# apapiu/transformer_latent_diffusion

Measured on AMD Instinct MI355X. Metric: images/sec (256px, 35-step CFG sampling), denoiser only, higher is better.
Workload: dtype bf16; 1 GPU; C1: 100M-param denoiser (d=768, L=12), 32x32x4 latents, 35 steps + CFG 6, DPM-Solver++(2M), 64 images/GPU (model batch 128); images_per_gpu=64, global_batch=64, n_iter=35, parallelism=single GPU

## Files before the change

### transformer_latent_diffusion_amd/csrc/tld_common.h

```cpp
#pragma once
#include <hip/hip_runtime.h>
#include <atomic>
#include <mutex>
#include <stdint.h>
#include "tld_gemm_plan.h"

namespace tld {

typedef __attribute__((ext_vector_type(8))) __bf16 bf16x8;
typedef __attribute__((ext_vector_type(4))) __bf16 bf16x4;
typedef __attribute__((ext_vector_type(2))) __bf16 bf16x2;
typedef __attribute__((ext_vector_type(16))) float f32x16;
typedef __attribute__((ext_vector_type(4))) float f32x4;
typedef __attribute__((ext_vector_type(4))) unsigned u32x4;
typedef __attribute__((ext_vector_type(8))) int i32x8;
typedef __attribute__((ext_vector_type(2))) float f32x2;

constexpr int kWave = 64;
constexpr int kHeadDim = 64;
constexpr float kLnEps = 1e-5f;

template <int CTRL>
__device__ __forceinline__ float dpp_add(float v) {
    const int s = __builtin_amdgcn_update_dpp(0, __float_as_int(v), CTRL, 0xf, 0xf, true);
// ... 222 lines not shown
    }
    return c;
}

enum : int {
    EP_EMBED_PLAIN = 0, EP_EMBED_MFMA = 1 , EP_LN_Q4 = 5 , EP_LN_GENERIC = 9, EP_LN_MX8 = 10,
    EP_QKV_ATTN = 11, EP_QKV_LN = 12, EP_QKV_PLAIN = 13,
    EP_ATT_256 = 14, EP_ATT_CHUNKED = 15, EP_ATT_64 = 17 , EP_ATT_MASKED = 19,
    EP_CROSS_MFMA = 20 , EP_CROSS_GPW1 = 24, EP_CROSS_GPWN = 25, EP_CROSS_VALU = 26, EP_CROSS_FANOUT = 27,
    EP_UP_FUSED16 = 28, EP_UP_FUSED32_SEAM = 29, EP_UP_FUSED16_SMALL = 30, EP_UP_PLAIN = 31, EP_DW_WHOLE = 32, EP_DW_TILED = 33, EP_DW_STREAM = 34,
    EP_DOWN_STATS = 35, EP_DOWN_NOSTATS = 36, EP_DOWN_MAIN = 37, EP_DOWN_SMALL64 = 38, EP_DOWN_SMALL128 = 39,
    EP_SPLITK4 = 40, EP_SPLITK8 = 41, EP_SPLITK_SMALL = 42, EP_SPLITK_FINISH12 = 43, EP_SPLITK_FINISH6 = 44,
    EP_TAIL_MFMA = 45 , EP_TAIL_PLAIN = 49, EP_UPDATE = 50, EP_UPDATE_FROM = 51, EP_UPDATE_FROM_MASK = 52, EP_START_MIX = 53,
    EP_QUANT_MX8 = 54, EP_CROSS_F8 = 55, EP_DW_TILED_F8 = 56, EP_DW_STREAM_F8 = 57,
    EP_UPDATE_REQ = 58, EP_UPDATE_REQ_MASK = 59, EP_START_MIX_REQ = 60,
    EP_COUNT = 61
};
extern thread_local uint64_t* g_path_sink;
inline void note_path(int bit) { if (g_path_sink) *g_path_sink |= 1ull << bit; }

int launch_gemm(const GemmParams& p, int epilogue, hipStream_t s);
void launch_updw_pp(const GemmParams& p, const GemmPlan& plan, hipStream_t s);
void launch_splitk_pp(const GemmParams& p, const GemmPlan& plan, hipStream_t s);
void launch_down_pp(const GemmParams& p, const GemmPlan& plan, hipStream_t s);
void launch_dwconv_seam(const uint32_t* seam, const uint32_t* dw_wpk, const float* dw_b_half, bf16* out, int ldo, int batch, int channels, hipStream_t s);
void launch_gemm_tn(const GemmParams& p, hipStream_t s);

void set_last_error(const char* msg);

void launch_quant_mx8(const bf16* in, uint8_t* out, uint8_t* scale, int M, int K, hipStream_t s);
// ... 50 lines not shown
    float* sa_out;
    int batch, ntok, d, heads;
};
void launch_cross_row(const CrossRowParams& p, hipStream_t s);
bool cross_row_supports_ln3_stats(int d);
bool splitk_resid_supported(int d);
void launch_splitk_resid(const float* parts, int nsplit, size_t slice_stride, const float* bias, resid_t* x, float2* stats_out, int M, int d, hipStream_t s);

struct TailParams {
    const resid_t* tok;
    const float* w;
    const bf16* w_hl;
    const float* b;
    float* out;
    int batch, C, S, p, grid, pd, d, ntok;
};
void launch_tail(const TailParams& p, hipStream_t s);

struct SamplerStepRow {
    float g, a, b, c, c1, c2;
    float s_next;
    int final_step;
};
struct SamplerStepParams {
    const float* x0_2b;
    float* x_t;
    float* x0_prev;
    float* out_latent;
    float* trace_x0; float* trace_xt;
    const float* noise;
    const float* z0;
    const float* mask;
// ... 25 lines not shown
```

### transformer_latent_diffusion_amd/csrc/tld_engine.hip

```cpp
#include "../../include/tld_hip.h"
#include "tld_common.h"
#include "tld_host.h"
#include "tld_refresh.h"

#include <cmath>
#include <cstdarg>
#include <cstdio>
#include <cstring>
#include <cstdlib>
#include <map>
#include <string>
#include <unordered_map>
#include <vector>

using namespace tld;

namespace {
thread_local char g_err[512] = "";
}
namespace tld {
void set_last_error(const char* msg) { snprintf(g_err, sizeof(g_err), "%s", msg); }
thread_local uint64_t* g_path_sink = nullptr;
}
namespace {
// ... 8 lines not shown
    tld_config cfg{};
    int d = 0, L = 0, H = 0, ntok = 0, grid = 0, pd = 0, hid = 0, img = 0, ne = 0, text = 0;
    bool finalized = false;
    bool fuse_dwconv = true;
    bool fp8 = false;
    bool fp8_fused = true;
    uint8_t *a8 = nullptr, *as8 = nullptr;
    std::map<std::string, HostTensor> host;

    float *angular = nullptr, *ff1_w = nullptr, *ff1_b = nullptr, *ff3_w = nullptr, *ff3_b = nullptr;
    float *label_w = nullptr, *label_b = nullptr, *norm_w = nullptr, *norm_b = nullptr;
    float *conv_w = nullptr, *conv_b = nullptr, *pln1_w = nullptr, *pln1_b = nullptr, *plin_wt = nullptr,
          *plin_b = nullptr, *pln2_w = nullptr, *pln2_b = nullptr, *pos = nullptr, *out_w = nullptr,
          *out_b = nullptr;
    bf16* out_w_hl = nullptr;
    bf16* plin_w_hl = nullptr;
    std::vector<Layer> layers;
    const float **tab_kv_w = nullptr, **tab_q_w = nullptr, **tab_n2_w = nullptr, **tab_n2_b = nullptr;
    RefreshPlan refresh;
    int64_t nparam = 0;

    resid_t* x = nullptr;
    resid_t* x_half = nullptr;
    bool share_l0 = true;
    bool guidance_skip = true;
    int64_t rows_cond = 0, rows_uncond = 0;
    bool fold_ln1 = true;
    bool low_latency = false;
    float* splitk = nullptr;
    int ll_split = 0;
// ... 119 lines not shown

#define SNAP(...) do { if (e->dbg_keep) { if (int _r = e->stages.copy(__VA_ARGS__)) return _r; } } while (0)
inline std::string blk_name(int l, const char* n) { return "blk" + std::to_string(l) + "." + n; }

inline bool eng_fused_qa(const tld_engine* e) { return e->fuse_qkv_attn && e->fold_ln1 && !e->fp8; }
inline bool eng_fuse_dw(const tld_engine* e) { return e->fuse_dwconv && (e->grid == 16 || (e->grid == 32 && e->seam)) && e->hid % 256 == 0; }

int reserve_snapshots(tld_engine* e) {
    const size_t B = (size_t)e->cfg.max_batch, M = B * e->ntok, d = e->d, hid = e->hid;
#define RES(name, bytes) do { if (int _r = e->stages.reserve(name, bytes)) return _r; } while (0)
    const size_t rs = sizeof(resid_t);
    RES("tokens0", M * d * rs); RES("out", B * e->img * 4);
    for (const char* n : {"step.x_t", "step.x0_prev", "step.x0", "step.x_next"}) RES(n, B * e->img * 4);
    RES("step.out", B * e->img * 4);
    for (int l = 0; l < e->L; ++l) {
        for (const char* n : {"x_in", "ca", "mlp"}) RES(blk_name(l, n), M * d * rs);
        RES(blk_name(l, "att"), M * d * 2); RES(blk_name(l, "sa"), M * d * 4);
        if (e->fold_ln1) RES(blk_name(l, "ln1"), M * kLnSlots * 8); else RES(blk_name(l, "xn1"), M * d * 2);
        if (!eng_fused_qa(e)) { RES(blk_name(l, "qk"), M * 2 * d * 2); RES(blk_name(l, "vt"), M * d * 2); }
        if (e->fold_ln3) RES(blk_name(l, "stats"), M * 8); else RES(blk_name(l, "xn3"), M * d * 2);
        if (!eng_fuse_dw(e)) RES(blk_name(l, "hid_pre"), M * hid * 2);
        if (e->fp8) {
            RES(blk_name(l, "a8_qkv.q"), M * d); RES(blk_name(l, "a8_qkv.s"), M * d / 32);
            RES(blk_name(l, "a8_up.q"), M * d); RES(blk_name(l, "a8_up.s"), M * d / 32);
            RES(blk_name(l, "a8_down.q"), M * hid); RES(blk_name(l, "a8_down.s"), M * hid / 32);
        }
        RES(blk_name(l, "hid"), M * hid * 2);
        if (e->splitk) RES(blk_name(l, "splitk"), (size_t)e->ll_split * M * d * 4);
    }
#undef RES
    for (int l = 0; l < e->L; ++l) {
// ... 196 lines not shown
                if (fold3) {
                    g.A = e->x; g.W = Ly.up_wf; g.bias = Ly.up_b1; g.ln_c1 = Ly.up_c1; g.row_stats = e->row_stats;
                }
#endif
                GEMM_TRY(blk_name(l, "up-projection"), launch_gemm(g, EPI_BIAS_BF16, s));
            }
            SNAP(blk_name(l, "hid_pre"), e->hid1, ST_BF16, s, M, e->hid);
            {
                ProfScope ps(e, KC_DWCONV, s);
                const bool dw8 = fuse8 && e->grid > 16;
                launch_dwconv_gelu(e->hid1, e->hid2, Ly.dw_w9c, Ly.dw_b, Ly.dw_w9c_half, Ly.dw_b_half, batch, e->grid, e->hid, s,
                                   dw8 ? e->a8 : nullptr, dw8 ? e->as8 : nullptr);
            }
        }
        if (!(fuse8 && e->grid > 16)) SNAP(blk_name(l, "hid"), e->hid2, ST_BF16, s, M, e->hid);
        if (e->low_latency && !e->fp8) {
            ProfScope ps(e, KC_GEMM_DOWN, s);
            GemmParams g{};
            g.A = e->hid2; g.lda = e->hid; g.W = Ly.down_w; g.ldw = e->hid; g.M = M; g.N = d; g.K = e->hid / e->ll_split; g.ksplit = e->ll_split;
            g.c_f32 = e->splitk; g.ldc = d;
            GEMM_TRY(blk_name(l, "split-K down projection"), launch_gemm(g, EPI_F32, s));
            SNAP(blk_name(l, "splitk"), e->splitk, ST_F32, s, e->ll_split, M, d);
            launch_splitk_resid(e->splitk, e->ll_split, (size_t)M * d, Ly.down_b, e->x, (fold1 && l + 1 < e->L) ? e->ln_stats : nullptr, M, d, s);
        } else
        {
            ProfScope ps(e, KC_GEMM_DOWN, s);
            GemmParams g{};
            g.A = e->hid2; g.lda = e->hid; g.W = Ly.down_w; g.ldw = e->hid; g.M = M; g.N = d; g.K = e->hid;
            g.bias = Ly.down_b; g.resid = e->x; g.ldr = d;
            g.stats_out = (fold1 && l + 1 < e->L) ? e->ln_stats : nullptr;
            if (e->fp8) {
                if (!(fuse8 && e->grid > 16)) launch_quant_mx8(e->hid2, e->a8, e->as8, M, e->hid, s);
                SNAP(blk_name(l, "a8_down.q"), e->a8, ST_U8, s, M, e->hid); SNAP(blk_name(l, "a8_down.s"), e->as8, ST_MX8S, s, M, e->hid / 32);
                g.f8 = 1; g.A = reinterpret_cast<const bf16*>(e->a8); g.W = reinterpret_cast<const bf16*>(Ly.down_w8);
                g.a_scale = e->as8; g.w_scale = Ly.down_s8;
            }
            GEMM_TRY(blk_name(l, "down projection"), launch_gemm(g, EPI_BIAS_RESID, s));
        }
        SNAP(blk_name(l, "mlp"), e->x, rdt, s, M, d);
    }
    {
        ProfScope ps(e, KC_TAIL, s);
        TailParams tp{};
        tp.tok = e->x; tp.w = e->out_w; tp.w_hl = e->out_w_hl; tp.b = e->out_b; tp.out = out; tp.batch = batch;
        tp.C = e->cfg.n_channels; tp.S = e->cfg.image_size; tp.p = e->cfg.patch_size; tp.grid = e->grid;
        tp.pd = e->pd; tp.d = d; tp.ntok = e->ntok;
        launch_tail(tp, s);
    }
    SNAP("out", out, ST_F32, s, batch, e->img);
    HIP_TRY(hipGetLastError());
    return TLD_OK;
}

struct SamplePlan {
    int B, n_max, stride;
    const tld_sample_request* requests;
    const float* coeffs;
    const float* guidance;
    int Tn; const float* sig; const int* noise_idx;
    const float *noise, *init_latent, *mask, *labels, *neg_labels;
    float sharp, bright;
// ... 194 lines not shown
    if (strncmp(prop.gcnArchName, "gfx950", 6) != 0)
        return fail(TLD_ERR_INVALID, "device %d is %s; this engine is built for gfx950 only", c->device_id, prop.gcnArchName);
    tld_engine* e = new tld_engine();
    e->cfg = *c;
    e->d = c->embed_dim; e->L = c->n_layers; e->H = c->embed_dim / 64; e->grid = grid; e->ntok = ntok;
    e->pd = pd; e->hid = c->mlp_multiplier * c->embed_dim; e->img = c->n_channels * c->image_size * c->image_size;
    e->ne = c->noise_embed_dims; e->text = c->text_emb_size;
    e->layers.resize(e->L);
    e->nparam = make_param_layout(e->d, e->L, e->ne, e->pd, e->hid, e->ntok, e->text).count;
    if (const char* fd = getenv("TLD_FUSE_DWCONV")) e->fuse_dwconv = atoi(fd) != 0;
    if (const char* sl = getenv("TLD_SHARE_L0")) e->share_l0 = atoi(sl) != 0;
    if (const char* gs = getenv("TLD_GUIDANCE_SKIP")) e->guidance_skip = atoi(gs) != 0;
    if (const char* f8 = getenv("TLD_FP8_FUSED")) e->fp8_fused = atoi(f8) != 0;
    if (const char* fl = getenv("TLD_FOLD_LN3")) e->fold_ln3 = atoi(fl) != 0;
    if (const char* fl = getenv("TLD_FOLD_LN1")) e->fold_ln1 = atoi(fl) != 0;
#ifndef TLD_RESID_BF16
    e->fold_ln3 = false;
    e->fold_ln1 = false;
#endif
    e->fold_ln1 = e->fold_ln1 && gemm_resid_stat_slots(e->d) > 0 && (3 * e->d) % 256 == 0;
    e->fold_ln3 = e->fold_ln3 && e->hid % 256 == 0 && cross_row_supports_ln3_stats(e->d);
    if (const char* fq = getenv("TLD_FUSE_QKV_ATTN")) e->fuse_qkv_attn = atoi(fq) != 0;
    e->fuse_qkv_attn = e->fuse_qkv_attn && e->fold_ln1 && ntok == 256 && e->d % 128 == 0;
    *out = e;
    return TLD_OK;
}

int tld_engine_load_tensor(tld_engine* e, const char* key, const void* host_ptr, const int64_t* shape,
                           int32_t ndim, int32_t dtype) {
    if (!e || !key || (!host_ptr && ndim > 0)) return fail(TLD_ERR_INVALID, "null argument");
    if (e->finalized) return fail(TLD_ERR_STATE, "weights already finalized");
// ... 209 lines not shown
                for (int64_t c = 0; c < hid; ++c) {
                    const uint32_t w0 = f32_to_bf16_rne(tr[(size_t)((du * 3 + 0) * hid + c)]);
                    const uint32_t w1 = f32_to_bf16_rne(tr[(size_t)((du * 3 + 1) * hid + c)]);
                    const uint32_t w2 = f32_to_bf16_rne(tr[(size_t)((du * 3 + 2) * hid + c)]);
                    pk[(size_t)((du * 4 + 0) * hid + c)] = w0 << 16;
                    pk[(size_t)((du * 4 + 1) * hid + c)] = w1 | (w2 << 16);
                    pk[(size_t)((du * 4 + 2) * hid + c)] = w0 | (w1 << 16);
                    pk[(size_t)((du * 4 + 3) * hid + c)] = w2;
                }
            if (int rc = dev_alloc(e, &Ly.dw_wpk, pk.size())) return rc;
            HIP_TRY(hipMemcpy(Ly.dw_wpk, pk.data(), pk.size() * sizeof(uint32_t), hipMemcpyHostToDevice));
            e->weight_bytes += (int64_t)pk.size() * 4;
        }
#undef LK
    }
    e->host.clear();
    {
        const size_t L = (size_t)e->L;
        std::vector<const float*> hk(L), hq(L), hg(L), hb(L);
        for (size_t l = 0; l < L; ++l) { hk[l] = e->layers[l].kv_w; hq[l] = e->layers[l].q_w; hg[l] = e->layers[l].n2_w; hb[l] = e->layers[l].n2_b; }
        const float** tabs = nullptr;
        if (int rc = dev_alloc(e, &tabs, 4 * L)) return rc;
        e->tab_kv_w = tabs; e->tab_q_w = tabs + L; e->tab_n2_w = tabs + 2 * L; e->tab_n2_b = tabs + 3 * L;
        HIP_TRY(hipMemcpy(e->tab_kv_w, hk.data(), L * sizeof(float*), hipMemcpyHostToDevice));
        HIP_TRY(hipMemcpy(e->tab_q_w, hq.data(), L * sizeof(float*), hipMemcpyHostToDevice));
        HIP_TRY(hipMemcpy(e->tab_n2_w, hg.data(), L * sizeof(float*), hipMemcpyHostToDevice));
        HIP_TRY(hipMemcpy(e->tab_n2_b, hb.data(), L * sizeof(float*), hipMemcpyHostToDevice));
    }
    {
        const ParamLayout pl = make_param_layout(e->d, e->L, e->ne, e->pd, e->hid, e->ntok, e->text);
// ... 2 lines not shown
        R.d = e->d; R.hid = e->hid; R.L = e->L; R.l0 = pl.layers[0]; R.layer_stride = pl.layer_stride();
        R.fold = e->fold_ln1 || e->fold_ln3; R.fp8 = e->fp8;
        Layer* ld = nullptr;
        if (int rc = dev_alloc(e, &ld, (size_t)e->L)) return rc;
        HIP_TRY(hipMemcpy(ld, e->layers.data(), (size_t)e->L * sizeof(Layer), hipMemcpyHostToDevice));
        R.layers_dev = ld;
        auto job = [&R](void* dst, int64_t src, int64_t n, int kind = RJ_COPY, int cols = 0) { if (dst) R.jobs[R.njobs++] = RefreshJob{dst, src, n, kind, cols}; };
        job(e->ff1_w, pl.ff1w, d * ne); job(e->ff1_b, pl.ff1b, d); job(e->ff3_w, pl.ff3w, d * d); job(e->ff3_b, pl.ff3b, d);
        job(e->label_w, pl.lbw, d * text); job(e->label_b, pl.lbb, d); job(e->norm_w, pl.nw, d); job(e->norm_b, pl.nb, d);
        job(e->conv_w, pl.cvw, pd * cpp); job(e->conv_b, pl.cvb, pd); job(e->pln1_w, pl.l1w, pd); job(e->pln1_b, pl.l1b, pd);
        job(e->plin_b, pl.lib, d); job(e->pln2_w, pl.l2w, d); job(e->pln2_b, pl.l2b, d); job(e->pos, pl.pos, N * d);
        job(e->out_w, pl.outw, pd * d); job(e->out_b, pl.outb, pd);
        job(e->out_w_hl, pl.outw, pd * d, RJ_SPLIT_HL); job(e->plin_w_hl, pl.liw, d * pd, RJ_SPLIT_HL);
        job(e->plin_wt, pl.liw, d * pd, RJ_TRANSPOSE, (int)pd);
        static_assert(kRefreshMaxJobs >= 21, "the images outside the blocks");
    }

    const size_t B2 = (size_t)e->cfg.max_batch, M = B2 * e->ntok;
    if (int rc = dev_alloc(e, &e->x, M * d)) return rc;
    if (int rc = dev_alloc(e, &e->x_half, M * d)) return rc;
    if (int rc = dev_alloc(e, &e->xn, M * d)) return rc;
    if (int rc = dev_alloc(e, &e->row_stats, M + 256)) return rc;
    if (int rc = dev_alloc(e, &e->ln_stats, (M + 256) * kLnSlots)) return rc;
    if (int rc = dev_alloc(e, &e->qk, M * 2 * d)) return rc;
    if (int rc = dev_alloc(e, &e->vt, M * d)) return rc;
    if (int rc = dev_alloc(e, &e->att, M * d)) return rc;
    if (int rc = dev_alloc(e, &e->hid1, M * hid)) return rc;
    if (e->grid == 32 && e->fuse_dwconv && hid % 256 == 0) { if (int rc = dev_alloc(e, &e->seam, M * hid / 4)) return rc; }
    if (int rc = dev_alloc(e, &e->hid2, M * hid)) return rc;
    if (e->fp8) {
// ... 552 lines not shown
```

### transformer_latent_diffusion_amd/csrc/tld_refresh.h

```cpp
#pragma once

#include "tld_param_layout.h"

namespace tld {

struct Layer {
    bf16 *qkv_w = nullptr, *up_w = nullptr, *down_w = nullptr;
    bf16 *qkv_wf = nullptr;
    float *qkv_c1 = nullptr, *qkv_b1 = nullptr;
    bf16 *qkv_wp = nullptr;
    float *qkv_c1p = nullptr, *qkv_b1p = nullptr;
    float *up_b = nullptr, *dw_w9c = nullptr, *dw_b = nullptr, *down_b = nullptr;
    float *dw_w9c_half = nullptr, *dw_b_half = nullptr;
    uint32_t* dw_wpk = nullptr;
    uint8_t *qkv_w8 = nullptr, *qkv_s8 = nullptr, *up_w8 = nullptr, *up_s8 = nullptr, *down_w8 = nullptr, *down_s8 = nullptr;
    bf16 *up_wf = nullptr;
    float *up_c1 = nullptr, *up_b1 = nullptr;
    float *n1_w = nullptr, *n1_b = nullptr, *n2_w = nullptr, *n2_b = nullptr, *n3_w = nullptr, *n3_b = nullptr;
    float *kv_w = nullptr, *q_w = nullptr;
};

enum { RJ_COPY = 0,
       RJ_SPLIT_HL = 1,
       RJ_TRANSPOSE = 2 };
struct RefreshJob { void* dst; int64_t src, n; int32_t kind, cols; };
constexpr int kRefreshMaxJobs = 24;

struct RefreshPlan {
    int d = 0, hid = 0, L = 0;
    const Layer* layers_dev = nullptr;
    LayerOffsets l0{};
    int64_t layer_stride = 0;
    bool fold = false, fp8 = false;
    RefreshJob jobs[kRefreshMaxJobs];
    int njobs = 0;
};

int launch_refresh_weights(const RefreshPlan& p, const float* flat, hipStream_t s);
void launch_quant_mx8_f32(const float* in, uint8_t* out, uint8_t* scale, int rows, int K, hipStream_t s);

}
```

### transformer_latent_diffusion_amd/csrc/tld_refresh.hip

```cpp
#include "tld_common.h"
#include "tld_stages.h"
#include "tld_refresh.h"
#include "tld_refresh_math.h"

namespace tld {

namespace {

struct RefreshJobs { RefreshJob job[kRefreshMaxJobs]; };

__device__ __forceinline__ uint16_t bf16_bits(float f) { return bf16_rne_bits(__float_as_uint(f)); }
__device__ __forceinline__ float bf16_value(uint16_t h) { return __uint_as_float((uint32_t)h << 16); }

__device__ __forceinline__ void copy_f32(float* __restrict__ dst, const float* __restrict__ src, int64_t n, int64_t tid, int64_t nth) {
    if (((reinterpret_cast<uintptr_t>(src) | reinterpret_cast<uintptr_t>(dst)) & 15) == 0 && (n & 3) == 0) {
        const float4* s4 = reinterpret_cast<const float4*>(src);
        float4* d4 = reinterpret_cast<float4*>(dst);
        for (int64_t i = tid; i < (n >> 2); i += nth) d4[i] = s4[i];
    } else {
        for (int64_t i = tid; i < n; i += nth) dst[i] = src[i];
    }
}

__device__ __forceinline__ void cast_bf16(uint16_t* __restrict__ dst, const float* __restrict__ src, int64_t n, int64_t tid, int64_t nth) {
// ... 123 lines not shown
            const float w = tile[lane][k];
            const float qf = bf16_value(bf16_bits(gs[k] * w));
            sc += (double)qf;
            sb += (double)bs[k] * (double)w;
        }
        __syncthreads();
    }
    const int n = row0 + lane;
    const float c1 = (float)sc;
    const float b1 = ln3 ? (float)(sb + (double)base[o.up_b + n]) : (float)sb;
    (ln3 ? Ly.up_c1 : Ly.qkv_c1)[n] = c1;
    (ln3 ? Ly.up_b1 : Ly.qkv_b1)[n] = b1;
    if (wp) { Ly.qkv_c1p[packed_row(lane)] = c1; Ly.qkv_b1p[packed_row(lane)] = b1; }
}

__device__ __forceinline__ void quant_mx8_f32_rows(const float* __restrict__ in, uint8_t* __restrict__ out, uint8_t* __restrict__ scale, int rows, int K,
                                                   int64_t tid, int64_t nth) {
    const int gpr = K >> 3;
    const int64_t groups = (int64_t)rows * gpr;
    const bool vec = (reinterpret_cast<uintptr_t>(in) & 15) == 0;
    for (int64_t g = tid; g < groups; g += nth) {
        const int row = (int)(g / gpr), k0 = (int)(g - (int64_t)row * gpr) * 8;
        const float* p = in + (int64_t)row * K + k0;
        float f[8];
        if (vec) {
            const float4 a = *reinterpret_cast<const float4*>(p), b = *reinterpret_cast<const float4*>(p + 4);
            f[0] = a.x; f[1] = a.y; f[2] = a.z; f[3] = a.w; f[4] = b.x; f[5] = b.y; f[6] = b.z; f[7] = b.w;
        } else {
#pragma unroll
            for (int e = 0; e < 8; ++e) f[e] = p[e];
// ... 33 lines not shown
    else if (blockIdx.y == 1) { if (Ly.up_w8) quant_mx8_f32_rows(base + o.up_w, Ly.up_w8, Ly.up_s8, hid, d, tid, nth); }
    else if (Ly.down_w8) quant_mx8_f32_rows(base + o.down_w, Ly.down_w8, Ly.down_s8, d, hid, tid, nth);
}

}

int launch_refresh_weights(const RefreshPlan& p, const float* flat, hipStream_t s) {
    RefreshJobs J{};
    for (int i = 0; i < p.njobs; ++i) J.job[i] = p.jobs[i];
    hipLaunchKernelGGL(refresh_globals_kernel, dim3(64, (unsigned)p.njobs), dim3(256), 0, s, J, flat);
    hipLaunchKernelGGL(refresh_layer_kernel, dim3(32, LJ_COUNT, (unsigned)p.L), dim3(256), 0, s, p.layers_dev, flat, p.l0, p.layer_stride, p.d, p.hid);
    if (p.fold) {
        const int rows = p.hid > 3 * p.d ? p.hid : 3 * p.d;
        hipLaunchKernelGGL(refresh_fold_kernel, dim3((unsigned)(rows / 64), 2, (unsigned)p.L), dim3(64), 0, s, p.layers_dev, flat, p.l0, p.layer_stride, p.d, p.hid);
    }
    if (p.fp8) hipLaunchKernelGGL(refresh_fp8_kernel, dim3(64, 3, (unsigned)p.L), dim3(256), 0, s, p.layers_dev, flat, p.l0, p.layer_stride, p.d, p.hid);
    const hipError_t e = hipGetLastError();
    if (e != hipSuccess) return fail(TLD_ERR_HIP, "weight refresh launch failed: %s", hipGetErrorString(e));
    return TLD_OK;
}

void launch_quant_mx8_f32(const float* in, uint8_t* out, uint8_t* scale, int rows, int K, hipStream_t s) {
    const int64_t groups = (int64_t)rows * (K >> 3);
    const unsigned blocks = (unsigned)((groups + 255) / 256 < 4096 ? (groups + 255) / 256 : 4096);
    hipLaunchKernelGGL(quant_mx8_f32_kernel, dim3(blocks), dim3(256), 0, s, in, out, scale, rows, K);
}

}
```

### transformer_latent_diffusion_amd/csrc/tld_rows.hip

```cpp
#include "tld_common.h"
#include <cstdlib>

namespace tld {

namespace {


template <int NJ, bool HALF>
__global__ __launch_bounds__(256) void embed_kernel(EmbedParams p) {
    extern __shared__ __attribute__((aligned(16))) char smem[];
    constexpr int d = NJ * 128 - (HALF ? 64 : 0);
    float* wt = reinterpret_cast<float*>(smem);
    float* cwt = wt + p.pd * d;
    for (int i = threadIdx.x; i < p.pd * d / 4; i += 256)
        reinterpret_cast<float4*>(wt)[i] = reinterpret_cast<const float4*>(p.lin_wt)[i];
    for (int i = threadIdx.x; i < p.pd * p.C * p.p * p.p; i += 256) {
        const int o = i / (p.C * p.p * p.p), k = i - o * (p.C * p.p * p.p);
        cwt[k * p.pd + o] = p.conv_w[i];
    }
    __syncthreads();
    const int lane = threadIdx.x & 63;
    const int wid = __builtin_amdgcn_readfirstlane(threadIdx.x >> 6);
    const bool live_last = !HALF || lane < 32;
    auto live = [&](int j) { return j + 1 < NJ || live_last; };
// ... 869 lines not shown
    if (row0 + tok >= total) return;
    const int b = row / p.ntok, tk = row - b * p.ntok;
    const int ti = tk / p.grid, tj = tk - ti * p.grid;
    const int pp = p.p * p.p;
#pragma unroll
    for (int t = 0; t < NT; ++t)
#pragma unroll
        for (int r = 0; r < 4; ++r) {
            const int f = t * 16 + 4 * kq + r;
            if (f < p.pd) {
                const int c = f / pp, uv = f - c * pp;
                const int u = uv / p.p, vv = uv - u * p.p;
                p.out[(((size_t)b * p.C + c) * p.S + (ti * p.p + u)) * p.S + (tj * p.p + vv)] = acc[t][r] + p.b[f];
            }
        }
}
#endif

template <bool MASK, int V, bool SLOT = false>
__global__ __launch_bounds__(256) void sampler_step_kernel(SamplerStepParams p) {
#pragma clang fp contract(off)
    const int i = (blockIdx.x * 256 + threadIdx.x) * V;
    const int n = p.active * p.img;
    if (i >= n) return;
    float cond[V], unc[V], prev[V], xin[V], eps[V], z[V], m[V], x0o[V], xto[V];
    auto load = [&](float* dst, const float* src) {
        if constexpr (V == 4) *reinterpret_cast<float4*>(dst) = *reinterpret_cast<const float4*>(src);
        else dst[0] = src[0];
    };
    auto store = [&](float* dst, const float* src) {
// ... 393 lines not shown
        const int slot = lane / GL;
        if ((lane & (GL - 1)) == 0 && slot < kLnSlots) stats_out[(size_t)row * kLnSlots + slot] = make_float2(su, sq);
    }
}

bool splitk_resid_supported(int d) { return d == 768 || d == 384; }

void launch_splitk_resid(const float* parts, int nsplit, size_t slice_stride, const float* bias, resid_t* x, float2* stats_out, int M, int d, hipStream_t s) {
    const dim3 grid((unsigned)((M + 3) / 4)), block(256);
    if (d == 768) { note_path(EP_SPLITK_FINISH12); hipLaunchKernelGGL(splitk_resid_kernel<12>, grid, block, 0, s, parts, nsplit, slice_stride, bias, x, stats_out, M); }
    else if (d == 384) { note_path(EP_SPLITK_FINISH6); hipLaunchKernelGGL(splitk_resid_kernel<6>, grid, block, 0, s, parts, nsplit, slice_stride, bias, x, stats_out, M); }
}

void launch_tail(const TailParams& p, hipStream_t s) {
#ifdef TLD_RESID_BF16
    if (p.w_hl && p.d % 128 == 0 && (long)p.pd * p.d <= 40960) {
        const int nt = (p.pd + 15) / 16, rows = p.batch * p.ntok;
        const int lds = 2 * nt * 16 * p.d * 2;
        dim3 grid((unsigned)((rows + 63) / 64));
#define TLD_TM(NT) do { TLD_LDS_OPT_IN((tail_mfma_kernel<NT>), lds); hipLaunchKernelGGL((tail_mfma_kernel<NT>), grid, dim3(256), lds, s, p, p.w_hl); } while (0)
        note_path(EP_TAIL_MFMA + (nt < 4 ? nt : 4) - 1);
        if (nt == 1) TLD_TM(1); else if (nt == 2) TLD_TM(2); else if (nt == 3) TLD_TM(3); else TLD_TM(4);
#undef TLD_TM
        return;
    }
#endif
    const int rpb = 64;
    const int rows = p.batch * p.ntok;
    const int lds = p.pd * p.d * (int)sizeof(float);
    note_path(EP_TAIL_PLAIN);
    TLD_DISPATCH_D(p.d, { TLD_LDS_OPT_IN((tail_kernel<NJ, HALF>), lds); hipLaunchKernelGGL((tail_kernel<NJ, HALF>), dim3((rows + rpb - 1) / rpb), dim3(256), lds, s, p, rpb); });
}

namespace {
bool aligned16(const void* a) { return (reinterpret_cast<uintptr_t>(a) & 15) == 0; }
}

void launch_sampler_step(const SamplerStepParams& p, int path, hipStream_t s, bool slots) {
    const int n = p.active * p.img;
    const bool vec = p.img % 4 == 0 && p.chan_stride % 4 == 0 && aligned16(p.x0_2b) && aligned16(p.x_t) && aligned16(p.x0_prev) && aligned16(p.out_latent) &&
                     aligned16(p.trace_x0) && aligned16(p.trace_xt) && aligned16(p.noise) && aligned16(p.z0) && aligned16(p.mask);
    const int threads = vec ? n / 4 : n;
    const dim3 grid((threads + 255) / 256), block(256);
    note_path(path);
    if (slots) {
        if (p.mask) {
            if (vec) hipLaunchKernelGGL((sampler_step_kernel<true, 4, true>), grid, block, 0, s, p);
// ... 249 lines not shown
```

### transformer_latent_diffusion_amd/denoiser.py

```python
from __future__ import annotations

import ctypes as C
import os
from collections import OrderedDict
from typing import Dict, Iterator, Optional

import numpy as np
import torch

from . import _lib
from .weights import param_count, param_layout, state_dict_spec, synth_state_dict

_IO_DTYPES = {torch.float32: _lib.DTYPE_F32, torch.bfloat16: _lib.DTYPE_BF16, torch.float16: _lib.DTYPE_F16}


class Denoiser:
    def __init__(self, image_size: int, noise_embed_dims: int, patch_size: int, embed_dim: int, dropout: float,
                 n_layers: int, text_emb_size: int = 768, mlp_multiplier: int = 4, n_channels: int = 4,
                 init_seed: int = 0):
        self.image_size = image_size
        self.noise_embed_dims = noise_embed_dims
        self.patch_size = patch_size
        self.embed_dim = embed_dim
        self.dropout = dropout
# ... 362 lines not shown
                U = schedule.guided_rows(sc, [steps[b] for b in order], skip)[0]
                return max(bi + u for bi, u in zip(schedule.active_prefix(sc), U))

            return self._run_sampler(noise, labels, n_max, trace, lambda h, B, eps, z0, m, lab, ng, out, tx0, txt, stream: _lib.check(
                _lib.lib().tld_sample_requests_guided(h, eps, z0, m, lab, ng, recs, table.ctypes.data_as(C.POINTER(C.c_float)),
                                                      gtab.ctypes.data_as(C.POINTER(C.c_float)), n_max, float(sharp_f), float(bright_f), out, B, tx0,
                                                      txt, stream), "tld_sample_requests_guided"),
                init_latents=init_latents, mask=mask, neg_labels=neg, order=order, new_trace=torch.zeros, model_batch=model_batch)
        return self._run_sampler(noise, labels, n_max, trace, lambda h, B, eps, z0, m, lab, ng, out, tx0, txt, stream: _lib.check(
            _lib.lib().tld_sample_requests(h, eps, z0, m, lab, ng, recs, table.ctypes.data_as(C.POINTER(C.c_float)), n_max, float(sharp_f),
                                           float(bright_f), out, B, tx0, txt, stream), "tld_sample_requests"),
            init_latents=init_latents, mask=mask, neg_labels=neg, order=order, new_trace=torch.zeros)

    PATH_NAMES = ("embed plain", "embed_mfma<2>", "embed_mfma<4>", "embed_mfma<6>", "embed_mfma<8>", "layernorm q4<1>", "layernorm q4<2>", "layernorm q4<3>",
                  "layernorm q4<4>", "layernorm generic", "layernorm mx8", "QKV fused with attention", "QKV LayerNorm-1 fold", "QKV plain", "attention 256",
                  "attention chunked", None, "attention 64", None, "attention masked", "cross_row_mfma<1>", "cross_row_mfma<2>",
                  "cross_row_mfma<3>", "cross_row_mfma<4>", "cross_row gpw 1", "cross_row gpw > 1", "cross_row VALU", "cross_row x_in fan-out",
                  "up fused 16", "up fused 32 + seam", "up fused 16 4-wave", "up alone", "depthwise whole image", "depthwise tiled", "depthwise streaming",
                  "down with stats_out", "down without stats_out", "down 8-wave", "down 4-wave 64", "down 4-wave 128", "split-K x4", "split-K x8",
                  "split-K 4-wave", "split-K finisher<12>", "split-K finisher<6>", "tail_mfma<1>", "tail_mfma<2>", "tail_mfma<3>", "tail_mfma<4>", "tail plain",
                  "update", "update_from", "update_from masked", "start_mix")
    FP8_PATH_NAMES = {10: "layernorm mx8", 54: "fp8 separate quantisation pass", 55: "fp8 cross_row writer", 56: "fp8 depthwise tiled",
                      57: "fp8 depthwise streaming"}

    SAMPLER_PATH_NAMES = {58: "update_requests", 59: "update_requests masked", 60: "start_mix per request"}

    def sample_rows(self):
        c, u = C.c_int64(), C.c_int64()
        _lib.check(_lib.lib().tld_engine_sample_rows(self._engine, C.byref(c), C.byref(u)), "tld_engine_sample_rows")
        return int(c.value), int(u.value)

    def set_debug(self, enable: bool = True):
        _lib.check(_lib.lib().tld_engine_set_debug(self._engine, int(enable)), "tld_engine_set_debug")

    def set_debug_step(self, step: int):
# ... 38 lines not shown
```

Before: 307.8 images/s.

## Fold last block's MLP down projection into output projection tail

Precomputes a combined weight W_out·W_down and a merged bias, so the last block's down-projection GEMM and residual write are skipped. A new tail kernel consumes the concatenation [x, hid] and produces the output image directly, using hi/lo bf16 split MFMAs. This removes one large GEMM (M×hid→d) and the residual round-trip for the final layer. In exchange the tail now reads the hid activations (K = d+hid) instead of only d, and it needs an extra refresh kernel to rebuild the folded weights.

New measurement: 311.7 images/s, median of 6. 1.01x the previous value.

```diff
diff --git a/transformer_latent_diffusion_amd/csrc/tld_common.h b/transformer_latent_diffusion_amd/csrc/tld_common.h
--- a/transformer_latent_diffusion_amd/csrc/tld_common.h
+++ b/transformer_latent_diffusion_amd/csrc/tld_common.h
@@ -260,6 +260,7 @@
     EP_TAIL_MFMA = 45 , EP_TAIL_PLAIN = 49, EP_UPDATE = 50, EP_UPDATE_FROM = 51, EP_UPDATE_FROM_MASK = 52, EP_START_MIX = 53,
     EP_QUANT_MX8 = 54, EP_CROSS_F8 = 55, EP_DW_TILED_F8 = 56, EP_DW_STREAM_F8 = 57,
     EP_UPDATE_REQ = 58, EP_UPDATE_REQ_MASK = 59, EP_START_MIX_REQ = 60,
+    EP_TAIL_FOLD = 16,
     EP_COUNT = 61
 };
 extern thread_local uint64_t* g_path_sink;
@@ -340,8 +341,15 @@
     const float* b;
     float* out;
     int batch, C, S, p, grid, pd, d, ntok;
+    const bf16* hid;
+    const bf16* wf_hl;
+    const float* bf;
+    int hidn;
 };
 void launch_tail(const TailParams& p, hipStream_t s);
+#ifdef TLD_RESID_BF16
+void launch_tail_fold_debug_row(float* row, const resid_t* x, const float* bias, int M, int d, hipStream_t s);
+#endif
 
 struct SamplerStepRow {
     float g, a, b, c, c1, c2;
diff --git a/transformer_latent_diffusion_amd/csrc/tld_engine.hip b/transformer_latent_diffusion_amd/csrc/tld_engine.hip
--- a/transformer_latent_diffusion_amd/csrc/tld_engine.hip
+++ b/transformer_latent_diffusion_amd/csrc/tld_engine.hip
@@ -2,6 +2,7 @@
 #include "tld_common.h"
 #include "tld_host.h"
 #include "tld_refresh.h"
+#include "tld_tail_fold_math.h"
 
 #include <cmath>
 #include <cstdarg>
@@ -46,6 +47,9 @@
           *plin_b = nullptr, *pln2_w = nullptr, *pln2_b = nullptr, *pos = nullptr, *out_w = nullptr,
           *out_b = nullptr;
     bf16* out_w_hl = nullptr;
+    bool fold_tail = true;
+    bf16* out_fold_hl = nullptr;
+    float* out_fold_b = nullptr;
     bf16* plin_w_hl = nullptr;
     std::vector<Layer> layers;
     const float **tab_kv_w = nullptr, **tab_q_w = nullptr, **tab_n2_w = nullptr, **tab_n2_b = nullptr;
@@ -195,7 +199,8 @@
     for (const char* n : {"step.x_t", "step.x0_prev", "step.x0", "step.x_next"}) RES(n, B * e->img * 4);
     RES("step.out", B * e->img * 4);
     for (int l = 0; l < e->L; ++l) {
-        for (const char* n : {"x_in", "ca", "mlp"}) RES(blk_name(l, n), M * d * rs);
+        for (const char* n : {"x_in", "ca"}) RES(blk_name(l, n), M * d * rs);
+        RES(blk_name(l, "mlp"), M * d * ((l + 1 == e->L && e->out_fold_hl) ? 4 : rs));
         RES(blk_name(l, "att"), M * d * 2); RES(blk_name(l, "sa"), M * d * 4);
         if (e->fold_ln1) RES(blk_name(l, "ln1"), M * kLnSlots * 8); else RES(blk_name(l, "xn1"), M * d * 2);
         if (!eng_fused_qa(e)) { RES(blk_name(l, "qk"), M * 2 * d * 2); RES(blk_name(l, "vt"), M * d * 2); }
@@ -422,7 +427,23 @@
             }
         }
         if (!(fuse8 && e->grid > 16)) SNAP(blk_name(l, "hid"), e->hid2, ST_BF16, s, M, e->hid);
-        if (e->low_latency && !e->fp8) {
+        const bool fold_tail = l + 1 == e->L && e->out_fold_hl && !e->fp8 && !e->low_latency;
+#ifdef TLD_RESID_BF16
+        if (fold_tail && e->dbg_keep) {
+            float* row = nullptr;
+            if (int rc = e->stages.sink(blk_name(l, "mlp"), M, d, &row)) return rc;
+            GemmParams g{};
+            g.A = e->hid2; g.lda = e->hid; g.W = Ly.down_w; g.ldw = e->hid; g.M = M; g.N = d; g.K = e->hid; g.c_f32 = row; g.ldc = d;
+            uint64_t* const sink = g_path_sink;
+            g_path_sink = nullptr;
+            const int rc = launch_gemm(g, EPI_F32, s);
+            g_path_sink = sink;
+            if (rc) { const std::string m = tld_last_error(); return fail(rc, "%s (debug row of the folded tail): %s", blk_name(l, "mlp").c_str(), m.c_str()); }
+            launch_tail_fold_debug_row(row, e->x, Ly.down_b, M, d, s);
+        }
+#endif
+        if (fold_tail) {
+        } else if (e->low_latency && !e->fp8) {
             ProfScope ps(e, KC_GEMM_DOWN, s);
             GemmParams g{};
             g.A = e->hid2; g.lda = e->hid; g.W = Ly.down_w; g.ldw = e->hid; g.M = M; g.N = d; g.K = e->hid / e->ll_split; g.ksplit = e->ll_split;
@@ -445,7 +466,7 @@
             }
             GEMM_TRY(blk_name(l, "down projection"), launch_gemm(g, EPI_BIAS_RESID, s));
         }
-        SNAP(blk_name(l, "mlp"), e->x, rdt, s, M, d);
+        if (!fold_tail) SNAP(blk_name(l, "mlp"), e->x, rdt, s, M, d);
     }
     {
         ProfScope ps(e, KC_TAIL, s);
@@ -453,6 +474,9 @@
         tp.tok = e->x; tp.w = e->out_w; tp.w_hl = e->out_w_hl; tp.b = e->out_b; tp.out = out; tp.batch = batch;
         tp.C = e->cfg.n_channels; tp.S = e->cfg.image_size; tp.p = e->cfg.patch_size; tp.grid = e->grid;
         tp.pd = e->pd; tp.d = d; tp.ntok = e->ntok;
+        if (e->out_fold_hl && !e->fp8 && !e->low_latency) {
+            tp.hid = e->hid2; tp.hidn = e->hid; tp.wf_hl = e->out_fold_hl; tp.bf = e->out_fold_b;
+        }
         launch_tail(tp, s);
     }
     SNAP("out", out, ST_F32, s, batch, e->img);
@@ -677,7 +701,9 @@
     if (const char* f8 = getenv("TLD_FP8_FUSED")) e->fp8_fused = atoi(f8) != 0;
     if (const char* fl = getenv("TLD_FOLD_LN3")) e->fold_ln3 = atoi(fl) != 0;
     if (const char* fl = getenv("TLD_FOLD_LN1")) e->fold_ln1 = atoi(fl) != 0;
+    if (const char* ft = getenv("TLD_FOLD_TAIL")) e->fold_tail = atoi(ft) != 0;
 #ifndef TLD_RESID_BF16
+    e->fold_tail = false;
     e->fold_ln3 = false;
     e->fold_ln1 = false;
 #endif
@@ -917,6 +943,30 @@
         }
 #undef LK
     }
+    if (e->fold_tail && !e->fp8) {
+        snprintf(key, sizeof(key), "denoiser_trans_block.decoder_blocks.%d.mlp.mlp.3.weight", e->L - 1);
+        const std::vector<float>& Wd = e->host[key].data;
+        snprintf(key, sizeof(key), "denoiser_trans_block.decoder_blocks.%d.mlp.mlp.3.bias", e->L - 1);
+        const std::vector<float>& bd = e->host[key].data;
+        const std::vector<float>& Wo = e->host["denoiser_trans_block.out_proj.0.weight"].data;
+        const std::vector<float>& bo = e->host["denoiser_trans_block.out_proj.0.bias"].data;
+        const int64_t pdp = tail_fold_padded_rows((int)pd), K = d + hid;
+        std::vector<uint16_t> img((size_t)(2 * pdp * K), 0);
+        std::vector<float> wf((size_t)hid), bf((size_t)pd);
+        std::vector<double> acc((size_t)hid);
+        for (int64_t f = 0; f < pd; ++f) {
+            const float* wo = &Wo[(size_t)(f * d)];
+            tail_fold_weight_row(wo, Wd.data(), (int)d, (int)hid, acc.data(), wf.data());
+            bf[(size_t)f] = tail_fold_bias(wo, bd.data(), bo[(size_t)f], (int)d);
+            for (int64_t k2 = 0; k2 < K; ++k2)
+                tail_fold_split(k2 < d ? wo[k2] : wf[(size_t)(k2 - d)], &img[(size_t)(f * K + k2)], &img[(size_t)((pdp + f) * K + k2)]);
+        }
+        if (int rc = dev_alloc(e, &e->out_fold_hl, img.size())) return rc;
+        if (int rc = dev_alloc(e, &e->out_fold_b, bf.size())) return rc;
+        HIP_TRY(hipMemcpy(e->out_fold_hl, img.data(), img.size() * 2, hipMemcpyHostToDevice));
+        HIP_TRY(hipMemcpy(e->out_fold_b, bf.data(), bf.size() * 4, hipMemcpyHostToDevice));
+        e->weight_bytes += (int64_t)img.size() * 2 + (int64_t)bf.size() * 4;
+    }
     e->host.clear();
     {
         const size_t L = (size_t)e->L;
@@ -949,6 +999,7 @@
         job(e->out_w_hl, pl.outw, pd * d, RJ_SPLIT_HL); job(e->plin_w_hl, pl.liw, d * pd, RJ_SPLIT_HL);
         job(e->plin_wt, pl.liw, d * pd, RJ_TRANSPOSE, (int)pd);
         static_assert(kRefreshMaxJobs >= 21, "the images outside the blocks");
+        R.tail_fold_hl = e->out_fold_hl; R.tail_fold_b = e->out_fold_b; R.outw = pl.outw; R.outb = pl.outb; R.pd = e->pd;
     }
 
     const size_t B2 = (size_t)e->cfg.max_batch, M = B2 * e->ntok;
diff --git a/transformer_latent_diffusion_amd/csrc/tld_refresh.h b/transformer_latent_diffusion_amd/csrc/tld_refresh.h
--- a/transformer_latent_diffusion_amd/csrc/tld_refresh.h
+++ b/transformer_latent_diffusion_amd/csrc/tld_refresh.h
@@ -34,6 +34,10 @@
     bool fold = false, fp8 = false;
     RefreshJob jobs[kRefreshMaxJobs];
     int njobs = 0;
+    bf16* tail_fold_hl = nullptr;
+    float* tail_fold_b = nullptr;
+    int64_t outw = 0, outb = 0;
+    int pd = 0;
 };
 
 int launch_refresh_weights(const RefreshPlan& p, const float* flat, hipStream_t s);
diff --git a/transformer_latent_diffusion_amd/csrc/tld_refresh.hip b/transformer_latent_diffusion_amd/csrc/tld_refresh.hip
--- a/transformer_latent_diffusion_amd/csrc/tld_refresh.hip
+++ b/transformer_latent_diffusion_amd/csrc/tld_refresh.hip
@@ -2,6 +2,7 @@
 #include "tld_stages.h"
 #include "tld_refresh.h"
 #include "tld_refresh_math.h"
+#include "tld_tail_fold_math.h"
 
 namespace tld {
 
@@ -161,6 +162,30 @@
     if (wp) { Ly.qkv_c1p[packed_row(lane)] = c1; Ly.qkv_b1p[packed_row(lane)] = b1; }
 }
 
+__global__ __launch_bounds__(256) void refresh_tail_fold_kernel(bf16* __restrict__ img_, float* __restrict__ bias, const float* __restrict__ wout,
+                                                                const float* __restrict__ bo, const float* __restrict__ wd, const float* __restrict__ bd,
+                                                                int pd, int d, int hid) {
+#pragma clang fp contract(off)
+    uint16_t* img = reinterpret_cast<uint16_t*>(img_);
+    const int K = d + hid;
+    const int64_t lo = (int64_t)tail_fold_padded_rows(pd) * K;
+    const int64_t nf = (int64_t)pd * hid, nw = (int64_t)pd * d;
+    const int64_t i = (int64_t)blockIdx.x * 256 + threadIdx.x;
+    if (i < nf + nw) {
+        int f, k;
+        float w;
+        if (i < nf) { f = (int)(i / hid); const int j = (int)(i - (int64_t)f * hid); k = d + j; w = tail_fold_weight(wout + (int64_t)f * d, wd, d, hid, j); }
+        else { const int64_t r = i - nf; f = (int)(r / d); k = (int)(r - (int64_t)f * d); w = wout[r]; }
+        uint16_t h, l;
+        tail_fold_split(w, &h, &l);
+        img[(int64_t)f * K + k] = h;
+        img[lo + (int64_t)f * K + k] = l;
+    } else if (i < nf + nw + pd) {
+        const int f = (int)(i - nf - nw);
+        bias[f] = tail_fold_bias(wout + (int64_t)f * d, bd, bo[f], d);
+    }
+}
+
 __device__ __forceinline__ void quant_mx8_f32_rows(const float* __restrict__ in, uint8_t* __restrict__ out, uint8_t* __restrict__ scale, int rows, int K,
                                                    int64_t tid, int64_t nth) {
     const int gpr = K >> 3;
@@ -224,6 +249,12 @@
         const int rows = p.hid > 3 * p.d ? p.hid : 3 * p.d;
         hipLaunchKernelGGL(refresh_fold_kernel, dim3((unsigned)(rows / 64), 2, (unsigned)p.L), dim3(64), 0, s, p.layers_dev, flat, p.l0, p.layer_stride, p.d, p.hid);
     }
+    if (p.tail_fold_hl) {
+        const float* last = flat + (int64_t)(p.L - 1) * p.layer_stride;
+        const int64_t items = (int64_t)p.pd * (p.hid + p.d + 1);
+        hipLaunchKernelGGL(refresh_tail_fold_kernel, dim3((unsigned)((items + 255) / 256)), dim3(256), 0, s, p.tail_fold_hl, p.tail_fold_b, flat + p.outw, flat + p.outb,
+                           last + p.l0.down_w, last + p.l0.down_b, p.pd, p.d, p.hid);
+    }
     if (p.fp8) hipLaunchKernelGGL(refresh_fp8_kernel, dim3(64, 3, (unsigned)p.L), dim3(256), 0, s, p.layers_dev, flat, p.l0, p.layer_stride, p.d, p.hid);
     const hipError_t e = hipGetLastError();
     if (e != hipSuccess) return fail(TLD_ERR_HIP, "weight refresh launch failed: %s", hipGetErrorString(e));
diff --git a/transformer_latent_diffusion_amd/csrc/tld_rows.hip b/transformer_latent_diffusion_amd/csrc/tld_rows.hip
--- a/transformer_latent_diffusion_amd/csrc/tld_rows.hip
+++ b/transformer_latent_diffusion_amd/csrc/tld_rows.hip
@@ -907,6 +907,111 @@
                 p.out[(((size_t)b * p.C + c) * p.S + (ti * p.p + u)) * p.S + (tj * p.p + vv)] = acc[t][r] + p.b[f];
             }
         }
+}
+
+template <int NT, int RT>
+__global__ __launch_bounds__(512) void tail_fold_kernel(TailParams p) {
+    extern __shared__ __attribute__((aligned(16))) char smem[];
+    f32x4* red = reinterpret_cast<f32x4*>(smem);
+    const int d = p.d, K = d + p.hidn, pdp = NT * 16;
+    const int lane = threadIdx.x & 63, wid = __builtin_amdgcn_readfirstlane(threadIdx.x >> 6);
+    const int tok = lane & 15, kq = lane >> 4;
+    const int total = p.batch * p.ntok;
+    const int row0 = blockIdx.x * (RT * 16);
+    const int nkb = K >> 5, dkb = d >> 5;
+    const int per = (nkb + 7) >> 3;
+    const int kb_lo = wid * per, kb_hi = kb_lo + per < nkb ? kb_lo + per : nkb;
+    unsigned xoff[RT], hoff[RT];
+#pragma unroll
+    for (int rt = 0; rt < RT; ++rt) {
+        const int r = row0 + rt * 16 + tok;
+        const unsigned row = (unsigned)(r < total ? r : total - 1);
+        xoff[rt] = row * (unsigned)d + kq * 8; hoff[rt] = row * (unsigned)p.hidn + kq * 8;
+    }
+    const bf16* wbase = p.wf_hl + (size_t)tok * K + kq * 8;
+    const size_t lo_plane = (size_t)pdp * K;
+    f32x4 acc[RT][NT];
+#pragma unroll
+    for (int rt = 0; rt < RT; ++rt)
+#pragma unroll
+        for (int t = 0; t < NT; ++t) acc[rt][t] = f32x4{0.f, 0.f, 0.f, 0.f};
+    constexpr int G = RT == 1 ? (NT == 1 ? 4 : NT == 2 ? 2 : 1) : 1;
+    bf16x8 xa[2][G][RT], wh[2][G][NT], wl[2][G][NT];
+    auto fetch = [&](int buf, int kb0) {
+#pragma unroll
+        for (int g = 0; g < G; ++g) {
+            int kb = kb0 + g;
+            kb = kb < nkb ? kb : nkb - 1;
+            const bool in_x = kb < dkb;
+            const int ko = (in_x ? kb : kb - dkb) * 32;
+#pragma unroll
+            for (int rt = 0; rt < RT; ++rt)
+                xa[buf][g][rt] = *reinterpret_cast<const bf16x8*>(in_x ? p.tok + xoff[rt] + ko : p.hid + hoff[rt] + ko);
+#pragma unroll
+            for (int t = 0; t < NT; ++t) {
+                const bf16* w = wbase + (size_t)t * 16 * K + kb * 32;
+                wh[buf][g][t] = *reinterpret_cast<const bf16x8*>(w);
+                wl[buf][g][t] = *reinterpret_cast<const bf16x8*>(w + lo_plane);
+            }
+        }
+    };
+    auto mma = [&](int buf, int kb0) {
+#pragma unroll
+        for (int g = 0; g < G; ++g) {
+            if (kb0 + g < kb_hi) {
+#pragma unroll
+                for (int rt = 0; rt < RT; ++rt)
+#pragma unroll
+                    for (int t = 0; t < NT; ++t) acc[rt][t] = __builtin_amdgcn_mfma_f32_16x16x32_bf16(wh[buf][g][t], xa[buf][g][rt], acc[rt][t], 0, 0, 0);
+#pragma unroll
+                for (int rt = 0; rt < RT; ++rt)
+#pragma unroll
+                    for (int t = 0; t < NT; ++t) acc[rt][t] = __builtin_amdgcn_mfma_f32_16x16x32_bf16(wl[buf][g][t], xa[buf][g][rt], acc[rt][t], 0, 0, 0);
+            }
+        }
+    };
+    fetch(0, kb_lo);
+    for (int kb0 = kb_lo; kb0 < kb_hi; kb0 += 2 * G) {
+        fetch(1, kb0 + G);
+        __builtin_amdgcn_sched_barrier(0);
+        mma(0, kb0);
+        __builtin_amdgcn_sched_barrier(0);
+        fetch(0, kb0 + 2 * G);
+        __builtin_amdgcn_sched_barrier(0);
+        mma(1, kb0 + G);
+        __builtin_amdgcn_sched_barrier(0);
+    }
+#pragma unroll
+    for (int rt = 0; rt < RT; ++rt)
+#pragma unroll
+        for (int t = 0; t < NT; ++t) red[(wid * (RT * NT) + rt * NT + t) * 64 + lane] = acc[rt][t];
+    __syncthreads();
+    const int pp = p.p * p.p;
+    for (int it = wid; it < RT * NT; it += 8) {
+        const int rt = it / NT, t = it - rt * NT;
+        f32x4 s[8];
+#pragma unroll
+        for (int w = 0; w < 8; ++w) s[w] = red[(w * (RT * NT) + it) * 64 + lane];
+        const f32x4 sum = ((s[0] + s[1]) + (s[2] + s[3])) + ((s[4] + s[5]) + (s[6] + s[7]));
+        const int row = row0 + rt * 16 + tok;
+        if (row >= total) continue;
+        const int b = row / p.ntok, tk = row - b * p.ntok;
+        const int ti = tk / p.grid, tj = tk - ti * p.grid;
+#pragma unroll
+        for (int r = 0; r < 4; ++r) {
+            const int f = t * 16 + 4 * kq + r;
+            if (f < p.pd) {
+                const int c = f / pp, uv = f - c * pp;
+                const int u = uv / p.p, vv = uv - u * p.p;
+                p.out[(((size_t)b * p.C + c) * p.S + (ti * p.p + u)) * p.S + (tj * p.p + vv)] = sum[r] + p.bf[f];
+            }
+        }
+    }
+}
+
+__global__ __launch_bounds__(256) void tail_fold_debug_row_kernel(float* __restrict__ row, const bf16* __restrict__ x, const float* __restrict__ bias, int64_t n, int d) {
+    const int64_t i = (int64_t)blockIdx.x * 256 + threadIdx.x;
+    if (i < n) row[i] = ((float)x[i] + row[i]) + bias[(int)(i % d)];
 }
 #endif
 
@@ -1330,6 +1435,21 @@
 
 void launch_tail(const TailParams& p, hipStream_t s) {
 #ifdef TLD_RESID_BF16
+    if (p.hid) {
+        const int nt = (p.pd + 15) / 16, rows = p.batch * p.ntok;
+        const int big = nt <= 2 ? 4 : 2;
+        const int rt = rows >= 16 * big * device_cu_count() ? big : 1;
+        const int lds = 8 * rt * nt * 1024;
+        dim3 grid((unsigned)((rows + 16 * rt - 1) / (16 * rt)));
+#define TLD_TF(NT, RT) hipLaunchKernelGGL((tail_fold_kernel<NT, RT>), grid, dim3(512), lds, s, p)
+        note_path(EP_TAIL_MFMA + nt - 1); note_path(EP_TAIL_FOLD);
+        if (nt == 1) { if (rt == 1) TLD_TF(1, 1); else TLD_TF(1, 4); }
+        else if (nt == 2) { if (rt == 1) TLD_TF(2, 1); else TLD_TF(2, 4); }
+        else if (nt == 3) { if (rt == 1) TLD_TF(3, 1); else TLD_TF(3, 2); }
+        else { if (rt == 1) TLD_TF(4, 1); else TLD_TF(4, 2); }
+#undef TLD_TF
+        return;
+    }
     if (p.w_hl && p.d % 128 == 0 && (long)p.pd * p.d <= 40960) {
         const int nt = (p.pd + 15) / 16, rows = p.batch * p.ntok;
         const int lds = 2 * nt * 16 * p.d * 2;
@@ -1347,6 +1467,13 @@
     note_path(EP_TAIL_PLAIN);
     TLD_DISPATCH_D(p.d, { TLD_LDS_OPT_IN((tail_kernel<NJ, HALF>), lds); hipLaunchKernelGGL((tail_kernel<NJ, HALF>), dim3((rows + rpb - 1) / rpb), dim3(256), lds, s, p, rpb); });
 }
+
+#ifdef TLD_RESID_BF16
+void launch_tail_fold_debug_row(float* row, const resid_t* x, const float* bias, int M, int d, hipStream_t s) {
+    const int64_t n = (int64_t)M * d;
+    hipLaunchKernelGGL(tail_fold_debug_row_kernel, dim3((unsigned)((n + 255) / 256)), dim3(256), 0, s, row, x, bias, n, d);
+}
+#endif
 
 namespace {
 bool aligned16(const void* a) { return (reinterpret_cast<uintptr_t>(a) & 15) == 0; }
diff --git a/transformer_latent_diffusion_amd/csrc/tld_tail_fold_math.h b/transformer_latent_diffusion_amd/csrc/tld_tail_fold_math.h
--- /dev/null
+++ b/transformer_latent_diffusion_amd/csrc/tld_tail_fold_math.h
@@ -0,0 +1,74 @@
+#pragma once
+
+#include <cstdint>
+#include <cstring>
+
+#include "tld_refresh_math.h"
+
+namespace tld {
+
+TLD_HD float tail_fold_f32_from_bits(uint32_t u) {
+#if defined(__HIP_DEVICE_COMPILE__)
+    return __uint_as_float(u);
+#else
+    float f;
+    memcpy(&f, &u, 4);
+    return f;
+#endif
+}
+TLD_HD uint32_t tail_fold_bits(float f) {
+#if defined(__HIP_DEVICE_COMPILE__)
+    return __float_as_uint(f);
+#else
+    uint32_t u;
+    memcpy(&u, &f, 4);
+    return u;
+#endif
+}
+
+TLD_HD void tail_fold_split(float w, uint16_t* hi, uint16_t* lo) {
+#if defined(__clang__)
+#pragma clang fp contract(off)
+#endif
+    const uint16_t h = bf16_rne_bits(tail_fold_bits(w));
+    *hi = h;
+    *lo = bf16_rne_bits(tail_fold_bits(w - tail_fold_f32_from_bits((uint32_t)h << 16)));
+}
+
+TLD_HD float tail_fold_weight(const float* wout_row, const float* wd, int d, int hid, int j) {
+#if defined(__clang__)
+#pragma clang fp contract(off)
+#endif
+    double s = 0.0;
+    for (int k = 0; k < d; ++k) {
+        const float q = tail_fold_f32_from_bits((uint32_t)bf16_rne_bits(tail_fold_bits(wd[(int64_t)k * hid + j])) << 16);
+        s += (double)wout_row[k] * (double)q;
+    }
+    return (float)s;
+}
+
+inline void tail_fold_weight_row(const float* wout_row, const float* wd, int d, int hid, double* acc, float* out) {
+#if defined(__clang__)
+#pragma clang fp contract(off)
+#endif
+    for (int j = 0; j < hid; ++j) acc[j] = 0.0;
+    for (int k = 0; k < d; ++k) {
+        const double w = (double)wout_row[k];
+        const float* row = wd + (int64_t)k * hid;
+        for (int j = 0; j < hid; ++j) acc[j] += w * (double)tail_fold_f32_from_bits((uint32_t)bf16_rne_bits(tail_fold_bits(row[j])) << 16);
+    }
+    for (int j = 0; j < hid; ++j) out[j] = (float)acc[j];
+}
+
+TLD_HD float tail_fold_bias(const float* wout_row, const float* bd, float bo, int d) {
+#if defined(__clang__)
+#pragma clang fp contract(off)
+#endif
+    double s = 0.0;
+    for (int k = 0; k < d; ++k) s += (double)wout_row[k] * (double)bd[k];
+    return (float)(s + (double)bo);
+}
+
+TLD_HD int tail_fold_padded_rows(int pd) { return (pd + 15) / 16 * 16; }
+
+}
diff --git a/transformer_latent_diffusion_amd/denoiser.py b/transformer_latent_diffusion_amd/denoiser.py
--- a/transformer_latent_diffusion_amd/denoiser.py
+++ b/transformer_latent_diffusion_amd/denoiser.py
@@ -400,11 +400,11 @@
 
     PATH_NAMES = ("embed plain", "embed_mfma<2>", "embed_mfma<4>", "embed_mfma<6>", "embed_mfma<8>", "layernorm q4<1>", "layernorm q4<2>", "layernorm q4<3>",
                   "layernorm q4<4>", "layernorm generic", "layernorm mx8", "QKV fused with attention", "QKV LayerNorm-1 fold", "QKV plain", "attention 256",
-                  "attention chunked", None, "attention 64", None, "attention masked", "cross_row_mfma<1>", "cross_row_mfma<2>",
+                  "attention chunked", "tail folded", "attention 64", None, "attention masked", "cross_row_mfma<1>", "cross_row_mfma<2>",
                   "cross_row_mfma<3>", "cross_row_mfma<4>", "cross_row gpw 1", "cross_row gpw > 1", "cross_row VALU", "cross_row x_in fan-out",
                   "up fused 16", "up fused 32 + seam", "up fused 16 4-wave", "up alone", "depthwise whole image", "depthwise tiled", "depthwise streaming",
                   "down with stats_out", "down without stats_out", "down 8-wave", "down 4-wave 64", "down 4-wave 128", "split-K x4", "split-K x8",
-                  "split-K 4-wave", "split-K finisher<12>", "split-K finisher<6>", "tail_mfma<1>", "tail_mfma<2>", "tail_mfma<3>", "tail_mfma<4>", "tail plain",
+                  "split-K 4-wave", "split-K finisher<12>", "split-K finisher<6>", "tail_mfma<1>", "tail_mfma<2>", "tail_mfma<3>", "tail_mfma<4>", None,
                   "update", "update_from", "update_from masked", "start_mix")
     FP8_PATH_NAMES = {10: "layernorm mx8", 54: "fp8 separate quantisation pass", 55: "fp8 cross_row writer", 56: "fp8 depthwise tiled",
                       57: "fp8 depthwise streaming"}
```
